# too-z/MultiModalPFN

Hardware: AMD Instinct MI355X
Metric: in-context rows/sec (support+query), PAD-UFES-20 shape, 1/2/4/8 MI355X (higher is better)
Workload: dtype f16

## Files before the change

### multimodalpfn_amd/csrc/featrow.hip

```cpp
#include <type_traits>

#include "common.h"
#include "kernels.h"

namespace mmpfn {

namespace {

constexpr int FR_E = 192;
constexpr int FR_H = 6;
constexpr int FR_ST = FEAT_IMG_STRIDE;
constexpr int FR_QKV_IMG = 96 * FR_ST;
constexpr int FR_PIECES = FR_QKV_IMG * 2 / 1024;

template <typename X8>
__device__ __forceinline__ X8 cat8(const f32x4& a, const f32x4& b, float s = 1.0f) {
  typedef decltype(X8{}[0]) T;
  X8 r;
#pragma unroll
  for (int i = 0; i < 4; ++i) r[i] = (T)(a[i] * s), r[4 + i] = (T)(b[i] * s);
  return r;
}

typedef __attribute__((address_space(3))) void lds_void;

#pragma clang diagnostic push
#pragma clang diagnostic ignored "-Winline-asm"
__device__ __forceinline__ void fr_dma16(uint32_t voff, const void* sbase, unsigned lds_dst) {
  asm volatile("s_mov_b32 m0, %2\n\ts_nop 0\n\tglobal_load_lds_dwordx4 %0, %1" ::"v"(voff), "s"(sbase), "s"(lds_dst)
               : "memory", "m0");
}
#pragma clang diagnostic pop

template <int NT, bool F16, bool LAST = false>
__global__ __launch_bounds__(256, NT <= 3 ? 2 : 1) void feat_rows_kernel(void* __restrict__ Xv,
                                                                         const void* __restrict__ packv, int S, int T,
                                                                         int M, float eps) {
  constexpr int Q0 = LAST ? NT - 1 : 0;
  typedef typename Op16<F16>::x8 X8;
  typedef std::conditional_t<F16, f16, float> XT;
  typedef typename Op16<F16>::t WT;
  const WT* __restrict__ pack = (const WT*)packv;
  __shared__ __attribute__((aligned(1024))) WT wbuf[2 * FR_QKV_IMG];
  const int tid = threadIdx.x, lane = tid & 63, wave = __builtin_amdgcn_readfirstlane(tid >> 6);
  const int n = lane & 15, g = lane >> 4;
  const int row = blockIdx.x * 4 + wave;
  const bool rowok = row < M * S;
  const int rc = rowok ? row : M * S - 1;
  const int mem = rc / S, sr = rc - mem * S;
  const int64_t SE = (int64_t)S * FR_E;
  XT* __restrict__ X = (XT*)Xv + (int64_t)mem * T * SE;

  const uint32_t dvoff = lane * 16;
  auto dma_wait = []() { asm volatile("s_waitcnt vmcnt(0)" ::: "memory"); };
  auto lds_u32 = [](const void* p) { return (unsigned)(uintptr_t)(lds_void*)p; };
  auto dma = [&](const void* srcv, void* dstv, int pieces) {
    const char* src = (const char*)srcv;
    const unsigned dst = lds_u32(dstv);
    for (int p = wave; p < pieces; p += 4)
      fr_dma16(dvoff, src + p * 1024, __builtin_amdgcn_readfirstlane(dst + p * 1024));
  };

  auto dma_piece = [&](const void* srcv, void* dstv, int i) {
    const int p = min(wave + 4 * i, FR_PIECES - 1);
    fr_dma16(dvoff, (const char*)srcv + p * 1024, __builtin_amdgcn_readfirstlane(lds_u32(dstv) + p * 1024));
  };
#ifndef FR_DMA_SPREAD
#define FR_DMA_SPREAD 1
#endif
  constexpr int FR_PPW = (FR_PIECES + 3) / 4;
  constexpr bool SPREAD = FR_DMA_SPREAD && F16;

  dma(pack, wbuf, FR_PIECES);
  const char* const xrow = (const char*)(X + (int64_t)sr * FR_E);
  uint32_t xoff[NT];
#pragma unroll
  for (int tt = 0; tt < NT; ++tt) {
    const int t = 16 * tt + n;
    xoff[tt] = (uint32_t)(((tt == NT - 1 && t >= T ? 0 : t) * SE + 8 * g) * sizeof(XT));
  }
  X8 xf[NT][FR_E / 32];
#pragma unroll
  for (int tt = 0; tt < NT; ++tt) {
    const int t = 16 * tt + n;
    const bool pad = tt == NT - 1 && t >= T;
#pragma unroll
    for (int ks = 0; ks < FR_E / 32; ++ks) {
      if constexpr (F16) {
        xf[tt][ks] = *(const f16x8*)(xrow + xoff[tt] + 64 * ks);
        if (pad) xf[tt][ks] = f16x8{};
      } else {
        const char* xr = xrow + xoff[tt] + 128 * ks;
        f32x4 lo = *(const f32x4*)xr, hi = *(const f32x4*)(xr + 16);
        if (pad) lo = hi = f32x4{0.f, 0.f, 0.f, 0.f};
        xf[tt][ks] = cat8<X8>(lo, hi);
      }
    }
  }
  dma_wait();
  __syncthreads();

  X8 of[FR_H][NT - Q0];
#pragma unroll
  for (int h = 0; h < FR_H; ++h) {
    const WT* nsrc = h + 1 < FR_H ? pack + (h + 1) * FR_QKV_IMG : pack + FR_H * FR_QKV_IMG;
    WT* ndst = h + 1 < FR_H ? wbuf + ((h + 1) & 1) * FR_QKV_IMG : wbuf;
    if constexpr (!SPREAD) dma(nsrc, ndst, FR_PIECES);
    const WT* wq = wbuf + (h & 1) * FR_QKV_IMG;

    X8 qf[NT], kf[NT];
#pragma unroll
    for (int j = 0; j < 2; ++j) {
      f32x4 qa[2][NT];
#pragma unroll
      for (int f = 0; f < 2; ++f)
#pragma unroll
        for (int tt = 0; tt < NT; ++tt) qa[f][tt] = f32x4{0.f, 0.f, 0.f, 0.f};
#pragma unroll
      for (int ks = 0; ks < FR_E / 32; ++ks) {
        X8 wqf[2];
#pragma unroll
        for (int f = 0; f < 2; ++f) wqf[f] = *(const X8*)(wq + (32 * j + 16 * f + n) * FR_ST + 32 * ks + 8 * g);
#pragma unroll
        for (int tt = 0; tt < NT; ++tt) {
          if (j == 0 && tt < Q0) continue;
#pragma unroll
          for (int f = 0; f < 2; ++f) qa[f][tt] = mfma16x(wqf[f], xf[tt][ks], qa[f][tt]);
        }
        if constexpr (SPREAD) {
          if (ks < FR_PPW / 2) dma_piece(nsrc, ndst, j * (FR_PPW / 2) + ks);
        }
      }
#pragma unroll
      for (int tt = 0; tt < NT; ++tt) (j == 0 ? qf[tt] : kf[tt]) = cat8<X8>(qa[0][tt], qa[1][tt]);
      __builtin_amdgcn_sched_barrier(0);
    }
    __builtin_amdgcn_sched_barrier(0);
    constexpr int NKP = (NT + 1) / 2;
    X8 vfr[2][NKP];
    {
      f32x4 va[2][NT];
#pragma unroll
      for (int f = 0; f < 2; ++f)
#pragma unroll
        for (int tt = 0; tt < NT; ++tt) va[f][tt] = f32x4{0.f, 0.f, 0.f, 0.f};
#pragma unroll
      for (int ks = 0; ks < FR_E / 32; ++ks) {
        X8 wvf[2];
#pragma unroll
        for (int f = 0; f < 2; ++f) wvf[f] = *(const X8*)(wq + (64 + 16 * f + n) * FR_ST + 32 * ks + 8 * g);
#pragma unroll
        for (int tt = 0; tt < NT; ++tt)
#pragma unroll
          for (int f = 0; f < 2; ++f) va[f][tt] = mfma16x(xf[tt][ks], wvf[f], va[f][tt]);
      }
#pragma unroll
      for (int mt = 0; mt < 2; ++mt)
#pragma unroll
        for (int kp = 0; kp < NKP; ++kp)
          vfr[mt][kp] = cat8<X8>(va[mt][2 * kp], 2 * kp + 1 < NT ? va[mt][2 * kp + 1] : f32x4{0.f, 0.f, 0.f, 0.f});
    }
    __builtin_amdgcn_sched_barrier(0);

#pragma unroll
    for (int qt = Q0; qt < NT; ++qt) {
      f32x4 st[NT];
#pragma unroll
      for (int kt = 0; kt < NT; ++kt) st[kt] = mfma16x(kf[kt], qf[qt], f32x4{0.f, 0.f, 0.f, 0.f});
#pragma unroll
      for (int i = 0; i < 4; ++i)
        if (16 * (NT - 1) + 4 * g + i >= T) st[NT - 1][i] = -INFINITY;
      float m = -INFINITY;
#pragma unroll
      for (int kt = 0; kt < NT; ++kt)
#pragma unroll
        for (int i = 0; i < 4; ++i) m = fmaxf(m, st[kt][i]);
      m = max_rows4(m);
      float sum = 0.f;
#pragma unroll
      for (int kt = 0; kt < NT; ++kt)
#pragma unroll
        for (int i = 0; i < 4; ++i) {
          const float e = __builtin_amdgcn_exp2f(st[kt][i] - m);
          st[kt][i] = e;
          sum += e;
        }
      const float inv = __builtin_amdgcn_rcpf(sum_rows4(sum));
      f32x4 oa[2] = {f32x4{0.f, 0.f, 0.f, 0.f}, f32x4{0.f, 0.f, 0.f, 0.f}};
#pragma unroll
      for (int kp = 0; kp < NKP; ++kp) {
        const X8 pb = cat8<X8>(st[2 * kp], 2 * kp + 1 < NT ? st[2 * kp + 1] : f32x4{0.f, 0.f, 0.f, 0.f});
#pragma unroll
        for (int mt = 0; mt < 2; ++mt) oa[mt] = mfma16x(vfr[mt][kp], pb, oa[mt]);
      }
      of[h][qt - Q0] = cat8<X8>(oa[0], oa[1], inv);
      __builtin_amdgcn_sched_barrier(0);
    }
    dma_wait();
    __syncthreads();
  }
  dma(pack + FR_H * FR_QKV_IMG + FR_QKV_IMG, wbuf + FR_QKV_IMG, FR_PIECES);
  dma_wait();
  __syncthreads();

#pragma unroll
  for (int tt = Q0; tt < NT; ++tt) {
    f32x4 y[FR_E / 16];
#pragma unroll
    for (int f = 0; f < FR_E / 16; ++f) {
      y[f] = f32x4{0.f, 0.f, 0.f, 0.f};
#pragma unroll
      for (int h = 0; h < FR_H; ++h)
        y[f] = mfma16x(*(const X8*)(wbuf + (16 * f + n) * FR_ST + 32 * h + 8 * g), of[h][tt - Q0], y[f]);
    }
    const int t = 16 * tt + n;
    const bool pad = tt == NT - 1 && t >= T;
    const bool valid = rowok && !pad && (!LAST || t == T - 1);
    char* const xr = (char*)xrow + xoff[tt] - 16 * g;
    float sm = 0.f;
    if constexpr (F16) {
#pragma unroll
      for (int f = 0; f < FR_E / 16; ++f)
#pragma unroll
        for (int i = 0; i < 4; ++i) {
          y[f][i] += (float)xf[tt][f >> 1][4 * (f & 1) + i];
          sm += y[f][i];
        }
    } else {
#pragma unroll
      for (int f = 0; f < FR_E / 16; ++f) {
        const f32x4 xv = *(const f32x4*)(xr + 64 * f);
#pragma unroll
        for (int i = 0; i < 4; ++i) {
          y[f][i] += xv[i];
          sm += y[f][i];
        }
      }
    }
    const float mean = sum_rows4(sm) * (1.0f / FR_E);
    float q = 0.f;
#pragma unroll
    for (int f = 0; f < FR_E / 16; ++f)
#pragma unroll
      for (int i = 0; i < 4; ++i) {
        const float dl = y[f][i] - mean;
        q += dl * dl;
      }
    const float rs = 1.0f / sqrtf(sum_rows4(q) * (1.0f / FR_E) + eps);
    if (valid) {
      if constexpr (F16) {
#pragma unroll
        for (int k = 0; k < FR_E / 32; ++k) {
          f16x8 ov;
#pragma unroll
          for (int i = 0; i < 4; ++i)
            ov[i] = (f16)((y[2 * k][i] - mean) * rs), ov[4 + i] = (f16)((y[2 * k + 1][i] - mean) * rs);
          *(f16x8*)(xrow + xoff[tt] + 64 * k) = ov;
        }
      } else {
#pragma unroll
        for (int f = 0; f < FR_E / 16; ++f) {
          f32x4 ov;
#pragma unroll
          for (int i = 0; i < 4; ++i) ov[i] = (y[f][i] - mean) * rs;
          *(f32x4*)(xr + 64 * f) = ov;
        }
      }
    }
  }
}

template <bool F16, bool LAST>
hipError_t launch_fr(void* X, const void* pk, int S, int T, int M, float eps, hipStream_t st) {
  const dim3 grid((M * S + 3) / 4), block(256);
  if (T <= 16) hipLaunchKernelGGL((feat_rows_kernel<1, F16, LAST>), grid, block, 0, st, X, pk, S, T, M, eps);
  else if (T <= 32) hipLaunchKernelGGL((feat_rows_kernel<2, F16, LAST>), grid, block, 0, st, X, pk, S, T, M, eps);
  else if (T <= 48) hipLaunchKernelGGL((feat_rows_kernel<3, F16, LAST>), grid, block, 0, st, X, pk, S, T, M, eps);
  else hipLaunchKernelGGL((feat_rows_kernel<4, F16, LAST>), grid, block, 0, st, X, pk, S, T, M, eps);
  return hipGetLastError();
}
}

hipError_t launch_feat_rows(void* X, const void* pack, int S, int T, int M, int E, int H, float eps, hipStream_t st,
                            DType x_t, bool last) {
  if (S <= 0 || M <= 0) return hipSuccess;
  if (E != FR_E || H != FR_H || T < 1 || T > 64 || x_t == DType::BF16) return hipErrorInvalidValue;
  if (last)
    return x_t == DType::F16 ? launch_fr<true, true>(X, pack, S, T, M, eps, st)
                             : launch_fr<false, true>(X, pack, S, T, M, eps, st);
  return x_t == DType::F16 ? launch_fr<true, false>(X, pack, S, T, M, eps, st)
                           : launch_fr<false, false>(X, pack, S, T, M, eps, st);
}

}
```

Measured before the change: 776,800.

## Restructure feature-row weight streaming into 32-row groups with register parking

Splits each head's QKV weight image into 32-row groups staged through either a six-slot or a three-slot LDS ring. The three-slot ring, with spilled attention outputs parked in LDS, is used for the NT=3 case to cut LDS use and registers so more blocks fit per CU. DMA issue is spread across the Q/K/V and output-projection loops, partial vmcnt waits replace full waits, and the output projection is processed in passes of one or two tiles with weights streamed per group. The intent is better occupancy and overlap of weight loads with MFMA work, at the cost of more barriers and more complex slot bookkeeping.

Result: faster. 794,400 (median of 6 runs) (+2.3%).

```diff
diff --git a/multimodalpfn_amd/csrc/featrow.hip b/multimodalpfn_amd/csrc/featrow.hip
--- a/multimodalpfn_amd/csrc/featrow.hip
+++ b/multimodalpfn_amd/csrc/featrow.hip
@@ -10,8 +10,17 @@
 constexpr int FR_E = 192;
 constexpr int FR_H = 6;
 constexpr int FR_ST = FEAT_IMG_STRIDE;
-constexpr int FR_QKV_IMG = 96 * FR_ST;
-constexpr int FR_PIECES = FR_QKV_IMG * 2 / 1024;
+constexpr int FR_GRP = 32 * FR_ST;
+constexpr int FR_GPIECES = FR_GRP * 2 / 1024;
+constexpr int FR_QKV_GRPS = 3 * FR_H;
+constexpr int FR_FRAG = 512;
+
+template <int NT, bool LAST>
+constexpr int fr_park(int h, int t) {
+  return NT == 3 && !LAST && t == 2 ? h : -1;
+}
+template <int NT, bool LAST>
+constexpr int FR_NPARK = NT == 3 && !LAST ? FR_H : 0;
 
 template <typename X8>
 __device__ __forceinline__ X8 cat8(const f32x4& a, const f32x4& b, float s = 1.0f) {
@@ -41,7 +50,9 @@
   typedef std::conditional_t<F16, f16, float> XT;
   typedef typename Op16<F16>::t WT;
   const WT* __restrict__ pack = (const WT*)packv;
-  __shared__ __attribute__((aligned(1024))) WT wbuf[2 * FR_QKV_IMG];
+  constexpr int NPARK = FR_NPARK<NT, LAST>;
+  constexpr int NSLOT = NPARK ? 3 : 6;
+  __shared__ __attribute__((aligned(1024))) WT wbuf[NSLOT * FR_GRP + 4 * NPARK * FR_FRAG];
   const int tid = threadIdx.x, lane = tid & 63, wave = __builtin_amdgcn_readfirstlane(tid >> 6);
   const int n = lane & 15, g = lane >> 4;
   const int row = blockIdx.x * 4 + wave;
@@ -52,26 +63,42 @@
   XT* __restrict__ X = (XT*)Xv + (int64_t)mem * T * SE;
 
   const uint32_t dvoff = lane * 16;
-  auto dma_wait = []() { asm volatile("s_waitcnt vmcnt(0)" ::: "memory"); };
   auto lds_u32 = [](const void* p) { return (unsigned)(uintptr_t)(lds_void*)p; };
-  auto dma = [&](const void* srcv, void* dstv, int pieces) {
-    const char* src = (const char*)srcv;
-    const unsigned dst = lds_u32(dstv);
-    for (int p = wave; p < pieces; p += 4)
-      fr_dma16(dvoff, src + p * 1024, __builtin_amdgcn_readfirstlane(dst + p * 1024));
-  };
-
-  auto dma_piece = [&](const void* srcv, void* dstv, int i) {
-    const int p = min(wave + 4 * i, FR_PIECES - 1);
-    fr_dma16(dvoff, (const char*)srcv + p * 1024, __builtin_amdgcn_readfirstlane(lds_u32(dstv) + p * 1024));
-  };
+  auto dma_piece = [&](int item, int p) {
+    const int grp = item < FR_QKV_GRPS + 6 ? item : item - 6;
+    const char* src = (const char*)(pack + grp * FR_GRP);
+    const unsigned dst = lds_u32(wbuf + (item % NSLOT) * FR_GRP);
+    fr_dma16(dvoff, src + p * 1024, __builtin_amdgcn_readfirstlane(dst + p * 1024));
+  };
+  auto dma_part = [&](int item, int i) { dma_piece(item, wave + 4 * i); };
+  auto dma_tail = [&](int item) {
+    if (wave == 0) dma_piece(item, FR_GPIECES - 1);
+  };
+  auto dma_grp = [&](int item) {
+#pragma unroll
+    for (int i = 0; i < 3; ++i) dma_part(item, i);
+    dma_tail(item);
+  };
+  auto dma_img = [&](int item0) {
+    for (int p = wave; p < 3 * FR_GPIECES; p += 4) dma_piece(item0, p);
+  };
+  auto dma_img_part = [&](int item0, int i) { dma_piece(item0, min(wave + 4 * i, 3 * FR_GPIECES - 1)); };
 #ifndef FR_DMA_SPREAD
 #define FR_DMA_SPREAD 1
 #endif
-  constexpr int FR_PPW = (FR_PIECES + 3) / 4;
   constexpr bool SPREAD = FR_DMA_SPREAD && F16;
-
-  dma(pack, wbuf, FR_PIECES);
+  auto dma_start = [&](int item) {
+    if constexpr (SPREAD) dma_tail(item);
+    else dma_grp(item);
+  };
+  auto sync_all = []() {
+    asm volatile("s_waitcnt vmcnt(0)" ::: "memory");
+    __syncthreads();
+  };
+  auto sync_but_last = []() { asm volatile("s_waitcnt vmcnt(3) lgkmcnt(0)\n\ts_barrier" ::: "memory"); };
+
+  if constexpr (NSLOT == 6) dma_img(0);
+  else dma_grp(0), dma_grp(1), dma_grp(2);
   const char* const xrow = (const char*)(X + (int64_t)sr * FR_E);
   uint32_t xoff[NT];
 #pragma unroll
@@ -97,17 +124,15 @@
       }
     }
   }
-  dma_wait();
-  __syncthreads();
-
-  X8 of[FR_H][NT - Q0];
+  sync_all();
+  if constexpr (NSLOT == 6 && !SPREAD) dma_img(3);
+
+  constexpr int NTQ = NT - Q0;
+  WT* const park = wbuf + 3 * FR_GRP + wave * (NPARK * FR_FRAG) + lane * 8;
+  X8 of[FR_H][NTQ];
 #pragma unroll
   for (int h = 0; h < FR_H; ++h) {
-    const WT* nsrc = h + 1 < FR_H ? pack + (h + 1) * FR_QKV_IMG : pack + FR_H * FR_QKV_IMG;
-    WT* ndst = h + 1 < FR_H ? wbuf + ((h + 1) & 1) * FR_QKV_IMG : wbuf;
-    if constexpr (!SPREAD) dma(nsrc, ndst, FR_PIECES);
-    const WT* wq = wbuf + (h & 1) * FR_QKV_IMG;
-
+    const WT* wimg = wbuf + ((3 * h) % NSLOT) * FR_GRP;
     X8 qf[NT], kf[NT];
 #pragma unroll
     for (int j = 0; j < 2; ++j) {
@@ -120,7 +145,7 @@
       for (int ks = 0; ks < FR_E / 32; ++ks) {
         X8 wqf[2];
 #pragma unroll
-        for (int f = 0; f < 2; ++f) wqf[f] = *(const X8*)(wq + (32 * j + 16 * f + n) * FR_ST + 32 * ks + 8 * g);
+        for (int f = 0; f < 2; ++f) wqf[f] = *(const X8*)(wimg + (32 * j + 16 * f + n) * FR_ST + 32 * ks + 8 * g);
 #pragma unroll
         for (int tt = 0; tt < NT; ++tt) {
           if (j == 0 && tt < Q0) continue;
@@ -128,12 +153,17 @@
           for (int f = 0; f < 2; ++f) qa[f][tt] = mfma16x(wqf[f], xf[tt][ks], qa[f][tt]);
         }
         if constexpr (SPREAD) {
-          if (ks < FR_PPW / 2) dma_piece(nsrc, ndst, j * (FR_PPW / 2) + ks);
+          if (NSLOT == 6 && ks < 5) dma_img_part(3 * h + 3, j * 5 + ks);
+          if (NSLOT == 3 && j == 0 && ks < 3 && h > 0) dma_part(3 * h + 2, ks);
         }
       }
 #pragma unroll
       for (int tt = 0; tt < NT; ++tt) (j == 0 ? qf[tt] : kf[tt]) = cat8<X8>(qa[0][tt], qa[1][tt]);
       __builtin_amdgcn_sched_barrier(0);
+    }
+    if constexpr (NSLOT == 3) {
+      sync_all();
+      dma_start(3 * h + 3), dma_start(3 * h + 4);
     }
     __builtin_amdgcn_sched_barrier(0);
     constexpr int NKP = (NT + 1) / 2;
@@ -148,11 +178,12 @@
       for (int ks = 0; ks < FR_E / 32; ++ks) {
         X8 wvf[2];
 #pragma unroll
-        for (int f = 0; f < 2; ++f) wvf[f] = *(const X8*)(wq + (64 + 16 * f + n) * FR_ST + 32 * ks + 8 * g);
+        for (int f = 0; f < 2; ++f) wvf[f] = *(const X8*)(wimg + (64 + 16 * f + n) * FR_ST + 32 * ks + 8 * g);
 #pragma unroll
         for (int tt = 0; tt < NT; ++tt)
 #pragma unroll
           for (int f = 0; f < 2; ++f) va[f][tt] = mfma16x(xf[tt][ks], wvf[f], va[f][tt]);
+        if constexpr (SPREAD && NSLOT == 3) dma_part(3 * h + 3 + ks / 3, ks % 3);
       }
 #pragma unroll
       for (int mt = 0; mt < 2; ++mt)
@@ -193,77 +224,110 @@
 #pragma unroll
         for (int mt = 0; mt < 2; ++mt) oa[mt] = mfma16x(vfr[mt][kp], pb, oa[mt]);
       }
-      of[h][qt - Q0] = cat8<X8>(oa[0], oa[1], inv);
+      const int ps = fr_park<NT, LAST>(h, qt);
+      if (ps >= 0) *(X8*)(park + ps * FR_FRAG) = cat8<X8>(oa[0], oa[1], inv);
+      else of[h][qt - Q0] = cat8<X8>(oa[0], oa[1], inv);
       __builtin_amdgcn_sched_barrier(0);
     }
-    dma_wait();
-    __syncthreads();
+    sync_all();
+    if constexpr (NSLOT == 3) {
+      if (h + 1 < FR_H) dma_start(3 * h + 5);
+      else dma_grp(3 * h + 5);
+    } else {
+      if (h + 1 == FR_H || !SPREAD) dma_img(3 * h + 6);
+    }
   }
-  dma(pack + FR_H * FR_QKV_IMG + FR_QKV_IMG, wbuf + FR_QKV_IMG, FR_PIECES);
-  dma_wait();
-  __syncthreads();
-
-#pragma unroll
-  for (int tt = Q0; tt < NT; ++tt) {
-    f32x4 y[FR_E / 16];
+  if constexpr (NSLOT == 6) sync_all();
+
+  constexpr int TPP = NT == 4 ? 1 : 2;
+  constexpr int NPASS = (NTQ + TPP - 1) / TPP, NITEM = FR_QKV_GRPS + 6 * (NSLOT == 3 ? NPASS : 1);
+#pragma unroll
+  for (int pass = 0; pass < NPASS; ++pass) {
+    const int t0 = Q0 + TPP * pass, nt = NT - t0 < TPP ? NT - t0 : TPP;
+    if constexpr (NPARK > 0) {
+#pragma unroll
+      for (int h = 0; h < FR_H; ++h)
+#pragma unroll
+        for (int k = 0; k < nt; ++k) {
+          const int ps = fr_park<NT, LAST>(h, t0 + k);
+          if (ps >= 0) of[h][t0 + k - Q0] = *(const X8*)(park + ps * FR_FRAG);
+        }
+    }
+    f32x4 y[TPP][FR_E / 16];
 #pragma unroll
     for (int f = 0; f < FR_E / 16; ++f) {
-      y[f] = f32x4{0.f, 0.f, 0.f, 0.f};
-#pragma unroll
-      for (int h = 0; h < FR_H; ++h)
-        y[f] = mfma16x(*(const X8*)(wbuf + (16 * f + n) * FR_ST + 32 * h + 8 * g), of[h][tt - Q0], y[f]);
-    }
-    const int t = 16 * tt + n;
-    const bool pad = tt == NT - 1 && t >= T;
-    const bool valid = rowok && !pad && (!LAST || t == T - 1);
-    char* const xr = (char*)xrow + xoff[tt] - 16 * g;
-    float sm = 0.f;
-    if constexpr (F16) {
+      const int item = FR_QKV_GRPS + (NSLOT == 3 ? 6 * pass : 0) + f / 2;
+      const int wrow = 32 * (item % NSLOT) + 16 * (f % 2);
+#pragma unroll
+      for (int k = 0; k < nt; ++k) y[k][f] = f32x4{0.f, 0.f, 0.f, 0.f};
+#pragma unroll
+      for (int h = 0; h < FR_H; ++h) {
+        const X8 w = *(const X8*)(wbuf + (wrow + n) * FR_ST + 32 * h + 8 * g);
+#pragma unroll
+        for (int k = 0; k < nt; ++k) y[k][f] = mfma16x(w, of[h][t0 + k - Q0], y[k][f]);
+      }
+      if (NSLOT == 3 && f % 2 == 1 && item + 1 < NITEM) {
+        if (item + 2 < NITEM) sync_but_last();
+        else sync_all();
+        if (item + 3 < NITEM) dma_grp(item + 3);
+      }
+    }
+    if constexpr (!F16) __builtin_amdgcn_sched_barrier(0);
+#pragma unroll
+    for (int k = 0; k < nt; ++k) {
+      const int tt = t0 + k;
+      const int t = 16 * tt + n;
+      const bool pad = tt == NT - 1 && t >= T;
+      const bool valid = rowok && !pad && (!LAST || t == T - 1);
+      char* const xr = (char*)xrow + xoff[tt] - 16 * g;
+      float sm = 0.f;
+      if constexpr (F16) {
+#pragma unroll
+        for (int f = 0; f < FR_E / 16; ++f)
+#pragma unroll
+          for (int i = 0; i < 4; ++i) {
+            y[k][f][i] += (float)xf[tt][f >> 1][4 * (f & 1) + i];
+            sm += y[k][f][i];
+          }
+      } else {
+#pragma unroll
+        for (int f = 0; f < FR_E / 16; ++f) {
+          const f32x4 xv = *(const f32x4*)(xr + 64 * f);
+#pragma unroll
+          for (int i = 0; i < 4; ++i) {
+            y[k][f][i] += xv[i];
+            sm += y[k][f][i];
+          }
+        }
+      }
+      const float mean = sum_rows4(sm) * (1.0f / FR_E);
+      float q = 0.f;
 #pragma unroll
       for (int f = 0; f < FR_E / 16; ++f)
 #pragma unroll
         for (int i = 0; i < 4; ++i) {
-          y[f][i] += (float)xf[tt][f >> 1][4 * (f & 1) + i];
-          sm += y[f][i];
-        }
-    } else {
-#pragma unroll
-      for (int f = 0; f < FR_E / 16; ++f) {
-        const f32x4 xv = *(const f32x4*)(xr + 64 * f);
-#pragma unroll
-        for (int i = 0; i < 4; ++i) {
-          y[f][i] += xv[i];
-          sm += y[f][i];
-        }
-      }
-    }
-    const float mean = sum_rows4(sm) * (1.0f / FR_E);
-    float q = 0.f;
-#pragma unroll
-    for (int f = 0; f < FR_E / 16; ++f)
-#pragma unroll
-      for (int i = 0; i < 4; ++i) {
-        const float dl = y[f][i] - mean;
-        q += dl * dl;
-      }
-    const float rs = 1.0f / sqrtf(sum_rows4(q) * (1.0f / FR_E) + eps);
-    if (valid) {
-      if constexpr (F16) {
-#pragma unroll
-        for (int k = 0; k < FR_E / 32; ++k) {
-          f16x8 ov;
-#pragma unroll
-          for (int i = 0; i < 4; ++i)
-            ov[i] = (f16)((y[2 * k][i] - mean) * rs), ov[4 + i] = (f16)((y[2 * k + 1][i] - mean) * rs);
-          *(f16x8*)(xrow + xoff[tt] + 64 * k) = ov;
-        }
-      } else {
-#pragma unroll
-        for (int f = 0; f < FR_E / 16; ++f) {
-          f32x4 ov;
-#pragma unroll
-          for (int i = 0; i < 4; ++i) ov[i] = (y[f][i] - mean) * rs;
-          *(f32x4*)(xr + 64 * f) = ov;
+          const float dl = y[k][f][i] - mean;
+          q += dl * dl;
+        }
+      const float rs = 1.0f / sqrtf(sum_rows4(q) * (1.0f / FR_E) + eps);
+      if (valid) {
+        if constexpr (F16) {
+#pragma unroll
+          for (int c = 0; c < FR_E / 32; ++c) {
+            f16x8 ov;
+#pragma unroll
+            for (int i = 0; i < 4; ++i)
+              ov[i] = (f16)((y[k][2 * c][i] - mean) * rs), ov[4 + i] = (f16)((y[k][2 * c + 1][i] - mean) * rs);
+            *(f16x8*)(xrow + xoff[tt] + 64 * c) = ov;
+          }
+        } else {
+#pragma unroll
+          for (int f = 0; f < FR_E / 16; ++f) {
+            f32x4 ov;
+#pragma unroll
+            for (int i = 0; i < 4; ++i) ov[i] = (y[k][f][i] - mean) * rs;
+            *(f32x4*)(xr + 64 * f) = ov;
+          }
         }
       }
     }
```
